# ALVI-Labs/frankenstein

Measured on AMD Instinct MI355X. Metric: neural frames/sec (train fwd+bwd+AdamW, whole job), higher is better.
Workload: dtype bf16; 1 GPU; brainformer-small (6L d=384 6x64 heads, N=6144 tokens) + 2-block perceiver, L1 head; fwd+bwd+clip+AdamW; per_gpu_batch=32, global_batch=32, frames_T=600, electrodes=256, parallelism=dp1, weights=random-init (seed 42)

## Files before the change

### frankenstein_amd/_lib.py

```python
from __future__ import annotations

import ctypes as C
from pathlib import Path

import os

LIB_PATH = Path(os.environ.get("FRANKEN_HIP_LIB") or Path(__file__).resolve().parent / "libfranken_hip.so")

FK_F32, FK_BF16 = 0, 1
MASK_NONE, MASK_CAUSAL, MASK_BLOCK_CAUSAL, MASK_PREFIX, MASK_KEYPAD, MASK_DENSE = 0, 1, 2, 3, 4, 5
NORM_LAYER, NORM_RMS = 0, 1
ATTN_Q_PRESCALED = 1

_p, _i64, _int, _f32, _f64, _sz, _u32 = C.c_void_p, C.c_int64, C.c_int, C.c_float, C.c_double, C.c_size_t, C.c_uint32

SIGNATURES = {
    "fk_version": (_int, []),
    "fk_last_error": (C.c_char_p, []),
    "fk_gemm_nt": (_int, [_p, _i64, _p, _i64, _p, _i64, _i64, _i64, _i64, _p, _p, _i64, _i64, _int, _int, _p]),
    "fk_gemm_nt_rope": (_int, [_p, _i64, _p, _i64, _p, _i64, _i64, _i64, _i64, _p, _p, _i64, _i64, _i64, _i64, _i64, _i64, _i64, _int, _p]),
    "fk_gemm_nt_swiglu": (_int, [_p, _i64, _p, _i64, _p, _i64, _p, _i64, _i64, _i64, _i64, _int, _p]),
    "fk_gemm_nt_dswiglu": (_int, [_p, _i64, _p, _i64, _p, _i64, _p, _i64, _i64, _i64, _i64, _int, _p]),
    "fk_mlp_bwd_fused": (_int, [_p, _i64, _p, _i64, _p, _i64, _p, _i64, _p, _i64, _p, _i64, _i64, _i64, _i64, _int, _p]),
    "fk_gemm_tn_workspace_bytes": (_sz, [_i64, _i64, _i64, _int]),
    "fk_gemm_tn": (_int, [_p, _i64, _p, _i64, _p, _i64, _i64, _i64, _i64, _int, _int, _p, _sz, _p]),
    "fk_colsum_workspace_bytes": (_sz, [_i64, _i64]),
    "fk_colsum": (_int, [_p, _i64, _p, _i64, _i64, _int, _int, _p, _sz, _p]),
    "fk_attn_fwd": (_int, [_p, _p, _p, _p, _p] + [_i64] * 13 + [_int, _i64, _i64, _i64, _p, _p, _f32, _int, _int, _p]),
    "fk_attn_bwd": (_int, [_p] * 10 + [_i64] * 13 + [_int, _i64, _i64, _i64, _p, _p, _f32, _p, _i64, _i64, _int, _int, _p]),
    "fk_attn_fwd_dropout": (_int, [_p, _p, _p, _p, _p] + [_i64] * 13 + [_int, _i64, _i64, _i64, _p, _p, _f32, _int, _f32, _p, _u32, _int, _p]),
    "fk_attn_bwd_dropout": (_int, [_p] * 10 + [_i64] * 13 + [_int, _i64, _i64, _i64, _p, _p, _f32, _p, _i64, _i64, _int, _f32, _p, _u32, _int, _p]),
    "fk_dropout": (_int, [_p, _p, _p, _i64, _f32, _p, _u32, _int, _p]),
    "fk_norm_fwd": (_int, [_p, _p, _p, _p, _p, _p, _i64, _i64, _f32, _int, _int, _p]),
    "fk_norm_bwd_workspace_bytes": (_sz, [_i64, _i64]),
    "fk_norm_bwd": (_int, [_p] * 9 + [_i64, _i64, _int, _int, _int, _p, _sz, _p]),
    "fk_rope": (_int, [_p, _i64, _i64, _i64, _i64, _i64, _p, _i64, _i64, _int, _int, _p]),
    "fk_patchify": (_int, [_p, _p, _i64, _i64, _i64, _i64, _i64, _int, _p]),
    "fk_swiglu_fwd": (_int, [_p, _p, _i64, _i64, _int, _p]),
    "fk_swiglu_bwd": (_int, [_p, _p, _p, _i64, _i64, _int, _p]),
    "fk_gelu_fwd": (_int, [_p, _p, _i64, _int, _p]),
    "fk_gelu_bwd": (_int, [_p, _p, _p, _i64, _int, _p]),
    "fk_cast_pack": (_int, [_p, _i64, _p, _i64, _i64, _i64, _int, _int, _p]),
    "fk_cast_pack_rows": (_int, [_p, _i64, _p, _i64, _i64, _i64, _int, _i64, _i64, _i64, _int, _p]),
    "fk_cast_pack_multi": (_int, [_p, _i64, _i64, _int, _p]),
    "fk_cast": (_int, [_p, _int, _p, _int, _i64, _p]),
# ... 68 lines not shown
```

### frankenstein_amd/csrc/mlp_fused.hip

```cpp
#include "fk_common.h"
#include <stdlib.h>

namespace {

#include "gemm_tile.h"

typedef __attribute__((address_space(3))) void lds_void_t;
typedef __attribute__((address_space(1))) const void glb_void_t;

struct MlpBwdArgs {
  const bf16_t* dy; const bf16_t* w2t; const bf16_t* h13; const bf16_t* w13t;
  bf16_t* dh13; bf16_t* dx;
  int64_t lddy, ldw2t, ldh, ldw13t, lddh, lddx;
  int M, H;
};

#ifndef MF_SPREAD
#define MF_SPREAD 1
#endif
#ifndef MF_SPREAD_ST
#define MF_SPREAD_ST 0
#endif
#ifndef MF_NT_DH13
#define MF_NT_DH13 1
// ... 449 lines not shown

  char* stg = smem + wave * 32 * MF_ROWP;
#pragma unroll
  for (int t = 0; t < MF_D / 32; ++t)
#pragma unroll
    for (int g = 0; g < 4; ++g) {
      bf16x4 v;
#pragma unroll
      for (int e = 0; e < 4; ++e) v[e] = (T)dx[t][4 * g + e];
      *reinterpret_cast<bf16x4*>(stg + li * MF_ROWP + (32 * t + 8 * g + 4 * lh) * 2) = v;
    }
  asm volatile("s_waitcnt lgkmcnt(0)" ::: "memory");
  if (lane < MF_D / 8) {
    for (int r = 0; r < 32; ++r) {
      const bf16x8 v = *reinterpret_cast<const bf16x8*>(stg + r * MF_ROWP + lane * 16);
      fk_st<true>(reinterpret_cast<bf16x8*>(p.dx + (int64_t)(m0w + r) * p.lddx + lane * 8), v);
    }
  }
  MF_ST(9)
  MF_ST_FLUSH
}


struct MlpUpArgs {
  const bf16_t* x; const bf16_t* w13; bf16_t* h13; bf16_t* g;
  int64_t ldx, ldw, ldh, ldg;
  int M, H;
};
constexpr int MU_NW = 8, MU_TOK = MU_NW * 32;
constexpr int MU_TILE = MF_KT * 32 * ROW_BYTES;
constexpr int MU_SLOT = 2 * MU_TILE;
constexpr int MU_HT = 32 * ROW_BYTES, MU_GT = 32 * 64;
constexpr int MU_LDS = 2 * MU_SLOT + MU_NW * (MU_HT + MU_GT);
static_assert(MU_LDS <= 160 * 1024, "LDS of a CU");
constexpr int MU_PIECES = MU_SLOT / 1024 / MU_NW;

__global__ __launch_bounds__(MU_NW * 64, 2) void mlp_up_fused_kernel(MlpUpArgs p) {
  extern __shared__ __attribute__((aligned(16))) char smem[];
  using T = bf16_t;
  const int tid = threadIdx.x, lane = tid & 63, li = lane & 31, lh = lane >> 5;
  const int wave = __builtin_amdgcn_readfirstlane(tid >> 6);
  const int m0w = blockIdx.x * MU_TOK + wave * 32;
  const int m = m0w + li, mc = m < p.M ? m : p.M - 1;
  const bool wave_full = m0w + 32 <= p.M;
  const int nchunks = p.H / 32, last = nchunks - 1;
  const int row8 = lane >> 3, ch = lane & 7;
  const unsigned lds0 = (unsigned)(uintptr_t)(lds_void_t*)smem;

  unsigned woff[MU_PIECES];
#pragma unroll
  for (int j = 0; j < MU_PIECES; ++j) {
    const int q = wave * MU_PIECES + j, tile = q / 24, s6 = (q % 24) >> 2, n = (q & 3) * 8 + row8;
    const int wrow = 8 * (n >> 2) + (n & 3) + 4 * tile;
    woff[j] = (unsigned)((wrow * (int)p.ldw + s6 * 64 + ((ch ^ ((n >> 1) & 7)) << 3)) * 2);
  }
  auto issue_w = [&](int c, int slot) __attribute__((always_inline)) {
    const void* gw = p.w13 + (int64_t)c * 64 * p.ldw;
    const unsigned d0 = __builtin_amdgcn_readfirstlane(lds0 + slot * MU_SLOT + wave * (MU_SLOT / MU_NW));
#pragma unroll
    for (int j = 0; j < MU_PIECES; ++j) mf_dma(gw, woff[j], d0 + j * 1024);
  };
  char* htile = smem + 2 * MU_SLOT + wave * (MU_HT + MU_GT);
  char* gtile = htile + MU_HT;
  T* hdst[4];
  T* gdst[2];
  bool hok[4], gok[2];
#pragma unroll
  for (int j = 0; j < 4; ++j) {
    const int mr = m0w + j * 8 + row8;
    hok[j] = mr < p.M;
    hdst[j] = p.h13 + (int64_t)(hok[j] ? mr : p.M - 1) * p.ldh + (ch << 3);
  }
#pragma unroll
  for (int j = 0; j < 2; ++j) {
    const int mr = m0w + j * 16 + (lane >> 2);
    gok[j] = mr < p.M;
    gdst[j] = p.g + (int64_t)(gok[j] ? mr : p.M - 1) * p.ldg + ((lane & 3) << 3);
  }

  issue_w(0, 0);
  Frag<T> xf[MF_D / 16];
  const T* xrow = p.x + (int64_t)mc * p.ldx + 8 * lh;
#pragma unroll
  for (int t = 0; t < MF_D / 16; ++t) frag_load_contig<T>(xf[t], xrow + 16 * t);
  asm volatile("s_waitcnt vmcnt(0)\n\ts_barrier" ::: "memory");

  bf16x8 rbh[4] = {}, rbg[2] = {};
  for (int c = 0; c < nchunks; ++c) {
    const char* t0 = smem + (c & 1) * MU_SLOT;
    const char* t1 = t0 + MU_TILE;
    if (c > 0) {
      if (wave_full) {
#pragma unroll
        for (int j = 0; j < 4; ++j) fk_st<true>(reinterpret_cast<bf16x8*>(hdst[j] + (c - 1) * 64), rbh[j]);
#pragma unroll
        for (int j = 0; j < 2; ++j) fk_st<true>(reinterpret_cast<bf16x8*>(gdst[j] + (c - 1) * 32), rbg[j]);
      } else {
#pragma unroll
        for (int j = 0; j < 4; ++j)
          if (hok[j]) fk_st<true>(reinterpret_cast<bf16x8*>(hdst[j] + (c - 1) * 64), rbh[j]);
#pragma unroll
        for (int j = 0; j < 2; ++j)
          if (gok[j]) fk_st<true>(reinterpret_cast<bf16x8*>(gdst[j] + (c - 1) * 32), rbg[j]);
      }
    }
    issue_w(c + 1 < nchunks ? c + 1 : last, (c + 1) & 1);
    f32x16 a1, a3;
#pragma unroll
// ... 43 lines not shown
    }
    asm volatile("s_waitcnt vmcnt(0)\n\ts_barrier" ::: "memory");
  }
  if (wave_full) {
#pragma unroll
    for (int j = 0; j < 4; ++j) fk_st<true>(reinterpret_cast<bf16x8*>(hdst[j] + last * 64), rbh[j]);
#pragma unroll
    for (int j = 0; j < 2; ++j) fk_st<true>(reinterpret_cast<bf16x8*>(gdst[j] + last * 32), rbg[j]);
  } else {
#pragma unroll
    for (int j = 0; j < 4; ++j)
      if (hok[j]) fk_st<true>(reinterpret_cast<bf16x8*>(hdst[j] + last * 64), rbh[j]);
#pragma unroll
    for (int j = 0; j < 2; ++j)
      if (gok[j]) fk_st<true>(reinterpret_cast<bf16x8*>(gdst[j] + last * 32), rbg[j]);
  }
}


struct QkvArgs {
  const bf16_t* x; const bf16_t* w; bf16_t* out; const float* table;
  int64_t ldx, ldw, ldo, table_bs, q_off;
  int M, N, T, pos_off, rot_chunks, q_chunks;
};
constexpr int QK_LDS = 2 * MU_SLOT + MU_NW * MU_HT;
static_assert(QK_LDS <= 160 * 1024, "LDS of a CU");

__global__ __launch_bounds__(MU_NW * 64, 2) void qkv_rope_fused_kernel(QkvArgs p) {
  extern __shared__ __attribute__((aligned(16))) char smem[];
  using T = bf16_t;
  const int tid = threadIdx.x, lane = tid & 63, li = lane & 31, lh = lane >> 5;
  const int wave = __builtin_amdgcn_readfirstlane(tid >> 6);
  const int m0w = blockIdx.x * MU_TOK + wave * 32;
  const int m = m0w + li, mc = m < p.M ? m : p.M - 1;
  const bool wave_full = m0w + 32 <= p.M;
  const int nchunks = p.N / 64, last = nchunks - 1;
  const int row8 = lane >> 3, ch = lane & 7;
  const unsigned lds0 = (unsigned)(uintptr_t)(lds_void_t*)smem;

  unsigned woff[MU_PIECES];
#pragma unroll
  for (int j = 0; j < MU_PIECES; ++j) {
    const int q = wave * MU_PIECES + j, tile = q / 24, s6 = (q % 24) >> 2, n = (q & 3) * 8 + row8;
    woff[j] = (unsigned)(((32 * tile + n) * (int)p.ldw + s6 * 64 + ((ch ^ ((n >> 1) & 7)) << 3)) * 2);
  }
  auto issue_w = [&](int c, int slot) __attribute__((always_inline)) {
    const void* gw = p.w + (int64_t)c * 64 * p.ldw;
    const unsigned d0 = __builtin_amdgcn_readfirstlane(lds0 + slot * MU_SLOT + wave * (MU_SLOT / MU_NW));
#pragma unroll
    for (int j = 0; j < MU_PIECES; ++j) mf_dma(gw, woff[j], d0 + j * 1024);
  };
  char* htile = smem + 2 * MU_SLOT + wave * MU_HT;
  T* odst[4];
  bool ook[4];
#pragma unroll
  for (int j = 0; j < 4; ++j) {
    const int mr = m0w + j * 8 + row8;
    ook[j] = mr < p.M;
    odst[j] = p.out + (int64_t)(ook[j] ? mr : p.M - 1) * p.ldo + (ch << 3);
  }
  const float* trow = p.table + (int64_t)(mc / p.T) * p.table_bs + (int64_t)(p.pos_off + mc % p.T) * 64 + 4 * lh;

  issue_w(0, 0);
  Frag<T> xf[MF_D / 16];
  const T* xrow = p.x + (int64_t)mc * p.ldx + 8 * lh;
#pragma unroll
  for (int t = 0; t < MF_D / 16; ++t) frag_load_contig<T>(xf[t], xrow + 16 * t);
  asm volatile("s_waitcnt vmcnt(0)\n\ts_barrier" ::: "memory");

  bf16x8 rb[4] = {};
  for (int c = 0; c < nchunks; ++c) {
    const char* t0 = smem + (c & 1) * MU_SLOT;
    const char* t1 = t0 + MU_TILE;
    if (c > 0) {
      if (wave_full) {
#pragma unroll
        for (int j = 0; j < 4; ++j) fk_st<true>(reinterpret_cast<bf16x8*>(odst[j] + (c - 1) * 64), rb[j]);
      } else {
#pragma unroll
        for (int j = 0; j < 4; ++j)
          if (ook[j]) fk_st<true>(reinterpret_cast<bf16x8*>(odst[j] + (c - 1) * 64), rb[j]);
      }
    }
    const bool rot = c < p.rot_chunks;
    f32x4 cs[8];
    if (rot) {
      const float* tq = trow + (c < p.q_chunks ? p.q_off : (int64_t)0);
      asm volatile("global_load_dwordx4 %0, %8, off\n\tglobal_load_dwordx4 %1, %8, off offset:32\n\t"
                   "global_load_dwordx4 %2, %8, off offset:64\n\tglobal_load_dwordx4 %3, %8, off offset:96\n\t"
                   "global_load_dwordx4 %4, %8, off offset:128\n\tglobal_load_dwordx4 %5, %8, off offset:160\n\t"
                   "global_load_dwordx4 %6, %8, off offset:192\n\tglobal_load_dwordx4 %7, %8, off offset:224"
// ... 44 lines not shown
#pragma unroll
    for (int j = 0; j < 4; ++j) rb[j] = *reinterpret_cast<const bf16x8*>(htile + nt_off(j * 8 + row8, ch));
    asm volatile("s_waitcnt vmcnt(0)\n\ts_barrier" ::: "memory");
  }
  if (wave_full) {
#pragma unroll
    for (int j = 0; j < 4; ++j) fk_st<true>(reinterpret_cast<bf16x8*>(odst[j] + last * 64), rb[j]);
  } else {
#pragma unroll
    for (int j = 0; j < 4; ++j)
      if (ook[j]) fk_st<true>(reinterpret_cast<bf16x8*>(odst[j] + last * 64), rb[j]);
  }
}

}

static bool mu_grid_fills(int64_t M) {
  const int64_t wg = fk_cdiv(M, MU_TOK), rounds = fk_cdiv(wg, 256);
  return wg * 10 >= rounds * 256 * 7;
}
bool fk_qkv_rope_fused_ok(int64_t M, int64_t N, int64_t K, int64_t lda, int64_t ldb, int64_t ldc, const void* bias, int64_t T, int64_t D, int64_t rot_cols,
                          int64_t q_cols, int dtype) {
  static const bool off = getenv("FK_QKV_FUSED") != nullptr && getenv("FK_QKV_FUSED")[0] == '0';
  return !off && dtype == FK_BF16 && K == MF_D && D == 64 && N % 64 == 0 && rot_cols % 64 == 0 && q_cols % 64 == 0 && rot_cols <= N && !bias && mu_grid_fills(M) &&
         M < (1LL << 31) && T > 0 && M % T == 0 && lda % 8 == 0 && ldb % 8 == 0 && ldc % 8 == 0 && 64 * ldb * 2 < (1LL << 32);
}
int fk_qkv_rope_fused_launch(const void* A, int64_t lda, const void* W, int64_t ldb, void* C, int64_t ldc, int64_t M, int64_t N, const float* table,
                             int64_t table_bs, int64_t T, int64_t pos_off, int64_t rot_cols, int64_t q_cols, int64_t q_off, void* stream) {
  QkvArgs a{(const bf16_t*)A, (const bf16_t*)W, (bf16_t*)C, table, lda, ldb, ldc, table_bs, q_off, (int)M, (int)N, (int)T, (int)pos_off,
            (int)(rot_cols / 64), (int)(q_cols / 64)};
  static bool once = (hipFuncSetAttribute(reinterpret_cast<const void*>(qkv_rope_fused_kernel), hipFuncAttributeMaxDynamicSharedMemorySize, QK_LDS) == hipSuccess);
  (void)once;
  hipLaunchKernelGGL(qkv_rope_fused_kernel, dim3((unsigned)fk_cdiv(M, MU_TOK)), dim3(MU_NW * 64), QK_LDS, (hipStream_t)stream, a);
  FK_CHECK_LAUNCH("fk_gemm_nt_rope (token-on-the-lane kernel)");
  return FK_OK;
}

bool fk_mlp_up_fused_ok(int64_t M, int64_t H, int64_t K, int64_t lda, int64_t ldb, int64_t ldh, int64_t ldg, int dtype) {
  static const bool off = getenv("FK_MLP_UP_FUSED") != nullptr && getenv("FK_MLP_UP_FUSED")[0] == '0';
  return !off && dtype == FK_BF16 && K == MF_D && H % 32 == 0 && mu_grid_fills(M) && M < (1LL << 31) && lda % 8 == 0 && ldb % 8 == 0 && ldh % 8 == 0 && ldg % 8 == 0 &&
         64 * ldb * 2 < (1LL << 32);
}
int fk_mlp_up_fused_launch(const void* A, int64_t lda, const void* W13, int64_t ldb, void* H13, int64_t ldh, void* G, int64_t ldg, int64_t M, int64_t H,
                           void* stream) {
  MlpUpArgs a{(const bf16_t*)A, (const bf16_t*)W13, (bf16_t*)H13, (bf16_t*)G, lda, ldb, ldh, ldg, (int)M, (int)H};
  static bool once = (hipFuncSetAttribute(reinterpret_cast<const void*>(mlp_up_fused_kernel), hipFuncAttributeMaxDynamicSharedMemorySize, MU_LDS) == hipSuccess);
  (void)once;
  hipLaunchKernelGGL(mlp_up_fused_kernel, dim3((unsigned)fk_cdiv(M, MU_TOK)), dim3(MU_NW * 64), MU_LDS, (hipStream_t)stream, a);
  FK_CHECK_LAUNCH("fk_gemm_nt_swiglu (token-on-the-lane kernel)");
  return FK_OK;
}

#ifdef MF_STAMP
extern "C" int fk_debug_mf_stamps(unsigned long long* out, int reset) {
  hipDeviceSynchronize();
  hipMemcpyFromSymbol(out, HIP_SYMBOL(mf_stamp_acc), sizeof(unsigned long long) * 16);
  if (reset) { unsigned long long z[16] = {0}; hipMemcpyToSymbol(HIP_SYMBOL(mf_stamp_acc), z, sizeof(z)); }
  return 0;
}
#endif

extern "C" int fk_mlp_bwd_fused(const void* dY, int64_t lddy, const void* W2T, int64_t ldw2t, const void* H13, int64_t ldh, const void* W13T,
                                int64_t ldw13t, void* dH13, int64_t lddh, void* dX, int64_t lddx, int64_t M, int64_t H, int64_t D, int dtype,
                                void* stream) {
  FK_CHECK_ARG(dtype == FK_BF16, "fk_mlp_bwd_fused: bf16 only (dtype %d)", dtype);
  FK_CHECK_ARG(D == MF_D, "fk_mlp_bwd_fused: model dimension %lld (built for %d)", (long long)D, MF_D);
  FK_CHECK_ARG(M > 0 && M < (1LL << 31) && H > 0 && H % 32 == 0 && H < (1 << 24), "fk_mlp_bwd_fused: bad shape M=%lld H=%lld", (long long)M, (long long)H);
  FK_CHECK_ARG(dY && W2T && H13 && W13T && dH13 && dX, "fk_mlp_bwd_fused: null pointer");
  FK_CHECK_ARG(lddy % 8 == 0 && ldw2t % 8 == 0 && ldh % 8 == 0 && ldw13t % 8 == 0 && lddh % 8 == 0 && lddx % 8 == 0 && lddy >= D && ldw2t >= D &&
                   ldh >= 2 * H && lddh >= 2 * H && ldw13t >= 2 * H && lddx >= D,
               "fk_mlp_bwd_fused: leading dimensions must be multiples of 8 elements and cover their rows");
  FK_CHECK_ARG(M * ldh * 2 < (1LL << 32) && (int64_t)D * ldw13t * 2 < (1LL << 32) && 32 * ldw2t * 2 < (1LL << 32),
               "fk_mlp_bwd_fused: the h13 block must be addressable with 32-bit byte offsets (M * ldh < 2^31 elements)");
// ... 16 lines not shown
```

### frankenstein_amd/engine.py

```python
from __future__ import annotations

from typing import List, Optional, Sequence, Tuple

import math
import os
import weakref

import torch

from . import kernels as K
from .kernels import Mask, NO_MASK

Tensor = torch.Tensor

_COMPUTE_DTYPE = torch.bfloat16
_EPOCH = 0


def set_compute_dtype(dtype) -> None:
    global _COMPUTE_DTYPE
    if isinstance(dtype, str):
        dtype = {"bf16": torch.bfloat16, "bfloat16": torch.bfloat16, "fp32": torch.float32, "float32": torch.float32}[dtype]
    assert dtype in (torch.bfloat16, torch.float32)
    _COMPUTE_DTYPE = dtype
# ... 319 lines not shown
class Dropout(torch.autograd.Function):

    @staticmethod
    def forward(ctx, x, drop):
        ctx.drop = drop
        return K.dropout(x.contiguous(), drop[0], drop[1], drop[2])

    @staticmethod
    def backward(ctx, dy):
        d = ctx.drop
        return K.dropout(dy.contiguous(), d[0], d[1], d[2]), None


class AttnBranch(torch.autograd.Function):

    @staticmethod
    def forward(ctx, x, ln_w, ln_b, pw, pb, qkv_b, spec, *qkv_w):
        H, D, mask, rope, residual, eps, nkind = spec[:7]
        drop = spec[7] if len(spec) > 7 else None
        B, N, d = x.shape
        M = B * N
        x2 = x.view(M, d)
        has_ln = ln_w is not None
        if has_ln:
            h, mean, rstd = K.norm_fwd(x2, ln_w.detach(), None if ln_b is None else ln_b.detach(), eps, nkind)
        else:
            h, mean, rstd = x2, None, None
        HD = H * D
        bq = None if qkv_b is None else shadow([qkv_b])
        prescale = False
        if rope is not None and D % 8 == 0 and (3 * HD) % 8 == 0:
            prescale = _attn_prescale(D) and mask.kind != K.MASK_DENSE and drop is None
            if prescale:
                tab, qtab = rope.pair((1.0 / math.sqrt(D)) * 1.4426950408889634)
                qkv = K.gemm_nt_rope(h, shadow(qkv_w), bq, tab, N, rope.pos_off(N), D, 2 * HD, q_cols=HD, q_table=qtab)
            else:
                qkv = K.gemm_nt_rope(h, shadow(qkv_w), bq, rope.table, N, rope.pos_off(N), D, 2 * HD)
            qkv3 = qkv.view(B, N, 3 * HD)
        elif (rope is None and N >= 64 and M % 8 == 0 and (3 * HD) % 8 == 0 and _attn_prescale(D) and mask.kind != K.MASK_DENSE and drop is None
              and os.environ.get("FK_ATTN_NO_IDENT_PRESCALE") is None):
            tab, qtab = identity_pair(D, (1.0 / math.sqrt(D)) * 1.4426950408889634, x.device)
            qkv = K.gemm_nt_rope(h, shadow(qkv_w), bq, tab, 8, 0, D, 2 * HD, q_cols=HD, q_table=qtab)
            qkv3 = qkv.view(B, N, 3 * HD)
            prescale = True
        else:
            qkv = K.gemm_nt(h, shadow(qkv_w), bias=bq)
            qkv3 = qkv.view(B, N, 3 * HD)
            if rope is not None:
                K.rope_(qkv3, 2 * H, D, rope.table, rope.pos_off(N))
        q, k, v = (qkv3[..., i * HD:(i + 1) * HD].unflatten(-1, (H, D)) for i in range(3))
        o, lse = K.attn_fwd(q, k, v, mask, q_prescaled=prescale, dropout=None if drop is None else drop[:3])
        if drop is None:
            y = K.gemm_nt(o.view(M, HD), shadow([pw]), bias=None if pb is None else shadow([pb]),
                          residual=x2 if residual else None)
        else:
            y = K.gemm_nt(o.view(M, HD), shadow([pw]), bias=None if pb is None else shadow([pb]))
            K.dropout(y, drop[0], drop[1], drop[3], residual=x2 if residual else None, out=y)
        ctx.spec, ctx.has_ln, ctx.nw, ctx.prescale = spec, has_ln, len(qkv_w), prescale
        ctx.flags = (ln_b is not None, pb is not None, qkv_b is not None)
        ctx.ln_b = ln_b
        ctx.save_for_backward(x, ln_w, pw, *qkv_w, h if has_ln else None, mean, rstd, qkv, o, lse)
        return y.view(B, N, -1)

    @staticmethod
    def backward(ctx, dy):
# ... 107 lines not shown
                       do.view(B, T, H, D), lse, dq.view(B, T, H, D), dkv3[..., :HD].unflatten(-1, (H, D)),
                       dkv3[..., HD:].unflatten(-1, (H, D)), mask)
        dh = K.gemm_nt(dq, shadow([qw], transpose=True))
        (dqw,) = wgrad(dq, h, [qw])
        dctx = K.gemm_nt(dkv, shadow([kw, vw], transpose=True))
        dkw, dvw = wgrad(dkv, c2, [kw, vw])
        dx, dg, db = norm_bwd(dh, x2, ln_w, ctx.ln_b, mean, rstd, dres=dy2)
        return dx.view(B, T, d), dctx.view(B, Nc, d), dg, db, dqw, dkw, dvw, dpw, None


_MLP_BWD_FUSED = os.environ.get("FK_MLP_BWD_FUSED", "1") != "0"


class MlpBranch(torch.autograd.Function):

    @staticmethod
    def forward(ctx, x, ln_w, ln_b, up_w, up_b, gate_w, down_w, down_b, spec):
        residual, eps, nkind = spec[:3]
        drop = spec[3] if len(spec) > 3 else None
        shp = x.shape
        d = shp[-1]
        x2 = x.reshape(-1, d)
        has_ln = ln_w is not None
        if has_ln:
            h, mean, rstd = K.norm_fwd(x2, ln_w.detach(), None if ln_b is None else ln_b.detach(), eps, nkind)
        else:
            h, mean, rstd = x2, None, None
        fused = gate_w is not None and up_b is None and up_w.shape[0] % 8 == 0
        if fused:
            a, g = K.gemm_nt_swiglu(h, shadow_swiglu(up_w, gate_w))
        else:
            ups = [up_w] if gate_w is None else [up_w, gate_w]
            a = K.gemm_nt(h, shadow(ups), bias=None if up_b is None else shadow([up_b]))
            g = K.gelu_fwd(a) if gate_w is None else K.swiglu_fwd(a)
        if drop is None:
            y = K.gemm_nt(g, shadow([down_w]), bias=None if down_b is None else shadow([down_b]),
                          residual=x2 if residual else None)
        else:
            y = K.gemm_nt(g, shadow([down_w]), bias=None if down_b is None else shadow([down_b]))
            K.dropout(y, drop[0], drop[1], drop[2], residual=x2 if residual else None, out=y)
        ctx.spec, ctx.has_ln, ctx.fused = spec, has_ln, fused
        ctx.flags = (ln_b is not None, up_b is not None, gate_w is not None, down_b is not None)
        ctx.ln_b = ln_b
        ctx.save_for_backward(x, ln_w, up_w, gate_w, down_w, h if has_ln else None, mean, rstd, a, g)
        return y.view(*shp[:-1], y.shape[-1])

    @staticmethod
    def backward(ctx, dy):
        residual, eps, nkind = ctx.spec[:3]
        drop = ctx.spec[3] if len(ctx.spec) > 3 else None
        x, ln_w, up_w, gate_w, down_w, h, mean, rstd, a, g = ctx.saved_tensors
        has_lnb, has_ub, gated, has_db = ctx.flags
        shp = x.shape
        d = shp[-1]
        x2 = x.reshape(-1, d)
        if h is None:
            h = x2
# ... 408 lines not shown
```

### frankenstein_amd/kernels.py

```python
from __future__ import annotations

import math
from typing import Optional, Tuple

import torch

from . import _lib
from ._lib import FK_BF16, FK_F32, MASK_BLOCK_CAUSAL, MASK_CAUSAL, MASK_DENSE, MASK_KEYPAD, MASK_NONE, MASK_PREFIX, NORM_LAYER, NORM_RMS, ATTN_Q_PRESCALED, call, lib

Tensor = torch.Tensor


TIMERS = None
TIMER_PREFIX = None


class _timed:
    __slots__ = ("name", "ev")

    def __init__(self, name):
        self.name = name

    def __enter__(self):
        self.ev = None
# ... 72 lines not shown
    q_off = 0
    if q_table is not None and q_cols:
        assert q_table.shape == table.shape and q_table.dtype == torch.float32 and q_table.is_contiguous() and q_table.stride() == table.stride()
        q_off = (q_table.data_ptr() - table.data_ptr()) // 4
    else:
        q_cols = 0
    with _timed(f"gemm_nt_rope:{M}x{N}x{Kd}"):
        call("fk_gemm_nt_rope", a.data_ptr(), a.stride(0), w.data_ptr(), w.stride(0), out.data_ptr(), N, M, N, Kd, _ptr(bias),
             table.data_ptr(), tbs, T, pos_off, D, rot_cols, q_cols, q_off, fk_dtype(a), _stream())
    return out


def gemm_nt_swiglu(a: Tensor, w13: Tensor) -> Tuple[Tensor, Tensor]:
    assert a.dim() == 2 and w13.dim() == 2 and a.shape[1] == w13.shape[1] and a.dtype == w13.dtype
    assert a.stride(1) == 1 and w13.is_contiguous()
    M, Kd = a.shape
    H = w13.shape[0] // 2
    h13 = torch.empty((M, 2 * H), dtype=a.dtype, device=a.device)
    g = torch.empty((M, H), dtype=a.dtype, device=a.device)
    with _timed(f"gemm_nt_swiglu:{M}x{2 * H}x{Kd}"):
        call("fk_gemm_nt_swiglu", a.data_ptr(), a.stride(0), w13.data_ptr(), w13.stride(0), h13.data_ptr(), 2 * H,
             g.data_ptr(), H, M, H, Kd, fk_dtype(a), _stream())
    return h13, g


def gemm_nt_dswiglu(dy: Tensor, w2t: Tensor, h13: Tensor) -> Tensor:
    assert dy.dim() == 2 and w2t.dim() == 2 and dy.shape[1] == w2t.shape[1] and dy.dtype == w2t.dtype == h13.dtype
    assert dy.stride(1) == 1 and w2t.is_contiguous() and h13.is_contiguous()
    M, Kd = dy.shape
    H = w2t.shape[0]
    assert h13.shape == (M, 2 * H)
    dh13 = torch.empty_like(h13)
    with _timed(f"gemm_nt_dswiglu:{M}x{H}x{Kd}"):
        call("fk_gemm_nt_dswiglu", dy.data_ptr(), dy.stride(0), w2t.data_ptr(), w2t.stride(0), h13.data_ptr(), 2 * H,
             dh13.data_ptr(), 2 * H, M, H, Kd, fk_dtype(dy), _stream())
    return dh13


def mlp_bwd_fused(dy: Tensor, w2t: Tensor, h13: Tensor, w13t: Tensor) -> Tuple[Tensor, Tensor]:
    M, d = dy.shape
    H = w2t.shape[0]
    assert dy.dtype == torch.bfloat16 == w2t.dtype == h13.dtype == w13t.dtype and dy.stride(1) == 1
    assert w2t.shape == (H, d) and w2t.is_contiguous() and h13.shape == (M, 2 * H) and h13.is_contiguous() and w13t.shape == (d, 2 * H) and w13t.is_contiguous()
    dh13 = torch.empty_like(h13)
    dx = torch.empty((M, d), dtype=dy.dtype, device=dy.device)
    with _timed(f"mlp_bwd_fused:{M}x{H}x{d}"):
# ... 567 lines not shown
```

### include/franken_hip.h

```cpp
#ifndef FRANKEN_HIP_H
#define FRANKEN_HIP_H

#include <stddef.h>
#include <stdint.h>

#ifdef __cplusplus
extern "C" {
#endif

#define FK_VERSION 302

#define FK_OK 0
#define FK_EINVAL (-1)
#define FK_ELAUNCH (-2)
#define FK_EUNSUPPORTED (-3)

enum { FK_F32 = 0, FK_BF16 = 1 };
enum { FK_MASK_NONE = 0, FK_MASK_CAUSAL = 1, FK_MASK_BLOCK_CAUSAL = 2, FK_MASK_PREFIX = 3, FK_MASK_KEYPAD = 4, FK_MASK_DENSE = 5 };
enum { FK_ATTN_Q_PRESCALED = 1 };
enum { FK_NORM_LAYER = 0, FK_NORM_RMS = 1 };
enum { FK_ACT_SWIGLU = 0, FK_ACT_GELU = 1 };

int fk_version(void);
const char* fk_last_error(void);

int fk_gemm_nt(const void* A, int64_t lda, const void* B, int64_t ldb, void* C, int64_t ldc, int64_t M, int64_t N,
               int64_t K, const void* bias, const void* residual, int64_t ldr, int64_t res_rows, int dtype,
               int out_dtype, void* stream);
int fk_gemm_nt_rope(const void* A, int64_t lda, const void* B, int64_t ldb, void* C, int64_t ldc, int64_t M, int64_t N,
                    int64_t K, const void* bias, const float* table, int64_t table_bs, int64_t T, int64_t pos_off, int64_t D,
                    int64_t rot_cols, int64_t q_cols, int64_t q_table_off, int dtype, void* stream);
int fk_gemm_nt_swiglu(const void* A, int64_t lda, const void* W13, int64_t ldb, void* H13, int64_t ldh, void* G,
                      int64_t ldg, int64_t M, int64_t H, int64_t K, int dtype, void* stream);
int fk_gemm_nt_dswiglu(const void* dY, int64_t lda, const void* W2T, int64_t ldb, const void* H13, int64_t ldh, void* dH13,
                       int64_t lddh, int64_t M, int64_t H, int64_t K, int dtype, void* stream);
int fk_mlp_bwd_fused(const void* dY, int64_t lddy, const void* W2T, int64_t ldw2t, const void* H13, int64_t ldh, const void* W13T,
                     int64_t ldw13t, void* dH13, int64_t lddh, void* dX, int64_t lddx, int64_t M, int64_t H, int64_t D, int dtype,
                     void* stream);
size_t fk_gemm_tn_workspace_bytes(int64_t M, int64_t N1, int64_t N2, int dtype);
int fk_gemm_tn(const void* A, int64_t lda, const void* B, int64_t ldb, float* C, int64_t ldc, int64_t M, int64_t N1,
               int64_t N2, int accumulate, int dtype, void* workspace, size_t workspace_bytes, void* stream);
size_t fk_colsum_workspace_bytes(int64_t rows, int64_t cols);
int fk_colsum(const void* X, int64_t ld, float* out, int64_t rows, int64_t cols, int accumulate, int dtype,
              void* workspace, size_t workspace_bytes, void* stream);

int fk_attn_fwd(const void* Q, const void* K, const void* V, void* O, float* LSE, int64_t B, int64_t H, int64_t Nq,
                int64_t Nk, int64_t D, int64_t q_bs, int64_t q_rs, int64_t k_bs, int64_t k_rs, int64_t v_bs,
                int64_t v_rs, int64_t o_bs, int64_t o_rs, int mask_kind, int64_t mask_c, int64_t q_off, int64_t k_off,
                const int32_t* limits, const int32_t* qfirst, float scale, int flags, int dtype, void* stream);
int fk_attn_bwd(const void* Q, const void* K, const void* V, const void* O, const void* dO, const float* LSE,
                void* dQ, void* dK, void* dV, float* delta_ws, int64_t B, int64_t H, int64_t Nq, int64_t Nk, int64_t D,
                int64_t q_bs, int64_t q_rs, int64_t k_bs, int64_t k_rs, int64_t v_bs, int64_t v_rs, int64_t o_bs,
                int64_t o_rs, int mask_kind, int64_t mask_c, int64_t q_off, int64_t k_off, const int32_t* limits,
                const int32_t* qfirst, float scale, const float* rope_table, int64_t rope_bs, int64_t rope_off, int flags,
                int dtype, void* stream);

int fk_attn_fwd_dropout(const void* Q, const void* K, const void* V, void* O, float* LSE, int64_t B, int64_t H, int64_t Nq,
                        int64_t Nk, int64_t D, int64_t q_bs, int64_t q_rs, int64_t k_bs, int64_t k_rs, int64_t v_bs,
// ... 118 lines not shown
```

Baseline: 393,400 frames/s.

## Fuse pre-norm LayerNorm/RMSNorm into QKV-rope and SwiGLU up-projection kernels

Adds templated LN variants of the token-on-the-lane QKV+rope and MLP up-projection kernels. Each one computes mean/rstd and the normalized activations in registers as a prologue, writes h/mean/rstd for backward, and feeds the normalized fragments straight into the GEMM. The engine routes pre-norm attention and SwiGLU MLP through these entry points when the input is contiguous. This removes a separate norm kernel launch and the re-read of h by the GEMM, at the cost of extra register and LDS pressure in the GEMM prologue.

```diff
diff --git a/frankenstein_amd/_lib.py b/frankenstein_amd/_lib.py
--- a/frankenstein_amd/_lib.py
+++ b/frankenstein_amd/_lib.py
@@ -21,6 +21,8 @@
     "fk_gemm_nt_rope": (_int, [_p, _i64, _p, _i64, _p, _i64, _i64, _i64, _i64, _p, _p, _i64, _i64, _i64, _i64, _i64, _i64, _i64, _int, _p]),
     "fk_gemm_nt_swiglu": (_int, [_p, _i64, _p, _i64, _p, _i64, _p, _i64, _i64, _i64, _i64, _int, _p]),
     "fk_gemm_nt_dswiglu": (_int, [_p, _i64, _p, _i64, _p, _i64, _p, _i64, _i64, _i64, _i64, _int, _p]),
+    "fk_norm_gemm_nt_rope": (_int, [_p, _p, _p, _f32, _int, _p, _p, _p, _p, _i64, _p, _i64, _i64, _i64, _i64, _p, _p, _i64, _i64, _i64, _i64, _i64, _i64, _i64, _int, _p]),
+    "fk_norm_gemm_nt_swiglu": (_int, [_p, _p, _p, _f32, _int, _p, _p, _p, _p, _i64, _p, _i64, _p, _i64, _i64, _i64, _i64, _int, _p]),
     "fk_mlp_bwd_fused": (_int, [_p, _i64, _p, _i64, _p, _i64, _p, _i64, _p, _i64, _p, _i64, _i64, _i64, _i64, _int, _p]),
     "fk_gemm_tn_workspace_bytes": (_sz, [_i64, _i64, _i64, _int]),
     "fk_gemm_tn": (_int, [_p, _i64, _p, _i64, _p, _i64, _i64, _i64, _i64, _int, _int, _p, _sz, _p]),
diff --git a/frankenstein_amd/csrc/mlp_fused.hip b/frankenstein_amd/csrc/mlp_fused.hip
--- a/frankenstein_amd/csrc/mlp_fused.hip
+++ b/frankenstein_amd/csrc/mlp_fused.hip
@@ -495,10 +495,101 @@
 }
 
 
+struct NormIn {
+  const float* gamma; const float* beta; bf16_t* h; float* mean; float* rstd;
+  float eps; int kind;
+};
+
+FK_DEV void mu_norm_params(const NormIn& n, int lane, f32x4 (&gb)[3]) {
+#pragma unroll
+  for (int r = 0; r < 3; ++r) {
+    const int q = lane + 64 * r;
+    gb[r] = f32x4{0.0f, 0.0f, 0.0f, 0.0f};
+    if (q < MF_D / 4) gb[r] = *reinterpret_cast<const f32x4*>(n.gamma + 4 * q);
+    else if (n.beta) gb[r] = *reinterpret_cast<const f32x4*>(n.beta + 4 * (q - MF_D / 4));
+  }
+}
+
+FK_DEV void mu_norm_prologue(Frag<bf16_t> (&xf)[MF_D / 16], const NormIn& n, const f32x4 (&gb)[3], char* tile, int lane, int m0w, int M) {
+  using T = bf16_t;
+  const int li = lane & 31, lh = lane >> 5, row8 = lane >> 3, ch = lane & 7;
+#pragma unroll
+  for (int r = 0; r < 3; ++r) *reinterpret_cast<f32x4*>(tile + 16 * (lane + 64 * r)) = gb[r];
+  const float inv = 1.0f / MF_D;
+  float s[8];
+#pragma unroll
+  for (int j = 0; j < 8; ++j) {
+    float a = 0.0f;
+#pragma unroll
+    for (int k = 0; k < 3; ++k)
+#pragma unroll
+      for (int i = 0; i < 8; ++i) a += (float)xf[j + 8 * k].v[i];
+    s[j] = a;
+  }
+#pragma unroll
+  for (int t = 0; t < MF_D / 16; ++t) asm volatile("" : "+v"(xf[t].v));
+  float c = ((s[0] + s[4]) + (s[2] + s[6])) + ((s[1] + s[5]) + (s[3] + s[7]));
+  const float mu = n.kind == FK_NORM_LAYER ? (c + __shfl_xor(c, 32, 64)) * inv : 0.0f;
+#pragma unroll
+  for (int j = 0; j < 8; ++j) {
+    float a = 0.0f;
+#pragma unroll
+    for (int k = 0; k < 3; ++k)
+#pragma unroll
+      for (int i = 0; i < 8; ++i) {
+        const float d = (float)xf[j + 8 * k].v[i] - mu;
+        a += d * d;
+      }
+    s[j] = a;
+  }
+#pragma unroll
+  for (int t = 0; t < MF_D / 16; ++t) asm volatile("" : "+v"(xf[t].v));
+  c = ((s[0] + s[4]) + (s[2] + s[6])) + ((s[1] + s[5]) + (s[3] + s[7]));
+  const float rs = rsqrtf((c + __shfl_xor(c, 32, 64)) * inv + n.eps);
+  const int m = m0w + li;
+  if (lh == 0 && m < M) {
+    if (n.mean) n.mean[m] = mu;
+    n.rstd[m] = rs;
+  }
+#pragma unroll
+  for (int t = 0; t < MF_D / 16; ++t) {
+    const char* gp = tile + (16 * t + 8 * lh) * 4;
+    const f32x4 g0 = *reinterpret_cast<const f32x4*>(gp), g1 = *reinterpret_cast<const f32x4*>(gp + 16);
+    const f32x4 b0 = *reinterpret_cast<const f32x4*>(gp + 4 * MF_D), b1 = *reinterpret_cast<const f32x4*>(gp + 4 * MF_D + 16);
+#pragma unroll
+    for (int i = 0; i < 8; ++i) {
+      float tt = ((float)xf[t].v[i] - mu) * rs;
+      if (n.kind == FK_NORM_RMS) tt = (float)(bf16_t)tt;
+      xf[t].v[i] = (T)(tt * (i < 4 ? g0[i] : g1[i - 4]) + (i < 4 ? b0[i] : b1[i - 4]));
+    }
+    if ((t & 3) == 3)
+      asm volatile("" : "+v"(xf[t - 3].v), "+v"(xf[t - 2].v), "+v"(xf[t - 1].v), "+v"(xf[t].v)::"memory");
+  }
+  T* hd[4];
+  bool hok[4];
+#pragma unroll
+  for (int j = 0; j < 4; ++j) {
+    const int mr = m0w + j * 8 + row8;
+    hok[j] = mr < M;
+    hd[j] = n.h + (int64_t)(hok[j] ? mr : M - 1) * MF_D + (ch << 3);
+  }
+#pragma unroll
+  for (int k = 0; k < MF_D / 64; ++k) {
+#pragma unroll
+    for (int tt = 0; tt < 4; ++tt) *reinterpret_cast<bf16x8*>(tile + nt_off(li, 2 * tt + lh)) = xf[4 * k + tt].v;
+#pragma unroll
+    for (int j = 0; j < 4; ++j) {
+      const bf16x8 v = *reinterpret_cast<const bf16x8*>(tile + nt_off(j * 8 + row8, ch));
+      if (hok[j]) fk_st<true>(reinterpret_cast<bf16x8*>(hd[j] + 64 * k), v);
+    }
+  }
+}
+
 struct MlpUpArgs {
   const bf16_t* x; const bf16_t* w13; bf16_t* h13; bf16_t* g;
   int64_t ldx, ldw, ldh, ldg;
   int M, H;
+  NormIn ln;
 };
 constexpr int MU_NW = 8, MU_TOK = MU_NW * 32;
 constexpr int MU_TILE = MF_KT * 32 * ROW_BYTES;
@@ -508,6 +599,7 @@
 static_assert(MU_LDS <= 160 * 1024, "LDS of a CU");
 constexpr int MU_PIECES = MU_SLOT / 1024 / MU_NW;
 
+template <bool LN>
 __global__ __launch_bounds__(MU_NW * 64, 2) void mlp_up_fused_kernel(MlpUpArgs p) {
   extern __shared__ __attribute__((aligned(16))) char smem[];
   using T = bf16_t;
@@ -552,11 +644,14 @@
   }
 
   issue_w(0, 0);
+  f32x4 gb[3];
+  if constexpr (LN) mu_norm_params(p.ln, lane, gb);
   Frag<T> xf[MF_D / 16];
   const T* xrow = p.x + (int64_t)mc * p.ldx + 8 * lh;
 #pragma unroll
   for (int t = 0; t < MF_D / 16; ++t) frag_load_contig<T>(xf[t], xrow + 16 * t);
   asm volatile("s_waitcnt vmcnt(0)\n\ts_barrier" ::: "memory");
+  if constexpr (LN) mu_norm_prologue(xf, p.ln, gb, htile, lane, m0w, p.M);
 
   bf16x8 rbh[4] = {}, rbg[2] = {};
   for (int c = 0; c < nchunks; ++c) {
@@ -646,10 +741,12 @@
   const bf16_t* x; const bf16_t* w; bf16_t* out; const float* table;
   int64_t ldx, ldw, ldo, table_bs, q_off;
   int M, N, T, pos_off, rot_chunks, q_chunks;
+  NormIn ln;
 };
 constexpr int QK_LDS = 2 * MU_SLOT + MU_NW * MU_HT;
 static_assert(QK_LDS <= 160 * 1024, "LDS of a CU");
 
+template <bool LN>
 __global__ __launch_bounds__(MU_NW * 64, 2) void qkv_rope_fused_kernel(QkvArgs p) {
   extern __shared__ __attribute__((aligned(16))) char smem[];
   using T = bf16_t;
@@ -686,11 +783,14 @@
   const float* trow = p.table + (int64_t)(mc / p.T) * p.table_bs + (int64_t)(p.pos_off + mc % p.T) * 64 + 4 * lh;
 
   issue_w(0, 0);
+  f32x4 gb[3];
+  if constexpr (LN) mu_norm_params(p.ln, lane, gb);
   Frag<T> xf[MF_D / 16];
   const T* xrow = p.x + (int64_t)mc * p.ldx + 8 * lh;
 #pragma unroll
   for (int t = 0; t < MF_D / 16; ++t) frag_load_contig<T>(xf[t], xrow + 16 * t);
   asm volatile("s_waitcnt vmcnt(0)\n\ts_barrier" ::: "memory");
+  if constexpr (LN) mu_norm_prologue(xf, p.ln, gb, htile, lane, m0w, p.M);
 
   bf16x8 rb[4] = {};
   for (int c = 0; c < nchunks; ++c) {
@@ -781,33 +881,84 @@
 bool fk_qkv_rope_fused_ok(int64_t M, int64_t N, int64_t K, int64_t lda, int64_t ldb, int64_t ldc, const void* bias, int64_t T, int64_t D, int64_t rot_cols,
                           int64_t q_cols, int dtype) {
   static const bool off = getenv("FK_QKV_FUSED") != nullptr && getenv("FK_QKV_FUSED")[0] == '0';
-  return !off && dtype == FK_BF16 && K == MF_D && D == 64 && N % 64 == 0 && rot_cols % 64 == 0 && q_cols % 64 == 0 && rot_cols <= N && !bias && mu_grid_fills(M) &&
-         M < (1LL << 31) && T > 0 && M % T == 0 && lda % 8 == 0 && ldb % 8 == 0 && ldc % 8 == 0 && 64 * ldb * 2 < (1LL << 32);
+  return !off && dtype == FK_BF16 && K == MF_D && D == 64 && N > 0 && N < (1LL << 31) && N % 64 == 0 && rot_cols % 64 == 0 && q_cols % 64 == 0 &&
+         rot_cols <= N && !bias && M > 0 && mu_grid_fills(M) && M < (1LL << 31) && T > 0 && M % T == 0 && lda % 8 == 0 && ldb % 8 == 0 && ldc % 8 == 0 &&
+         lda >= K && ldb >= K && ldc >= N && 64 * ldb * 2 < (1LL << 32);
+}
+template <bool LN> static int qkv_launch(const QkvArgs& a, void* stream) {
+  static bool once = (hipFuncSetAttribute(reinterpret_cast<const void*>(qkv_rope_fused_kernel<LN>), hipFuncAttributeMaxDynamicSharedMemorySize, QK_LDS) == hipSuccess);
+  (void)once;
+  hipLaunchKernelGGL(qkv_rope_fused_kernel<LN>, dim3((unsigned)fk_cdiv(a.M, MU_TOK)), dim3(MU_NW * 64), QK_LDS, (hipStream_t)stream, a);
+  FK_CHECK_LAUNCH("fk_gemm_nt_rope (token-on-the-lane kernel)");
+  return FK_OK;
 }
 int fk_qkv_rope_fused_launch(const void* A, int64_t lda, const void* W, int64_t ldb, void* C, int64_t ldc, int64_t M, int64_t N, const float* table,
                              int64_t table_bs, int64_t T, int64_t pos_off, int64_t rot_cols, int64_t q_cols, int64_t q_off, void* stream) {
   QkvArgs a{(const bf16_t*)A, (const bf16_t*)W, (bf16_t*)C, table, lda, ldb, ldc, table_bs, q_off, (int)M, (int)N, (int)T, (int)pos_off,
-            (int)(rot_cols / 64), (int)(q_cols / 64)};
-  static bool once = (hipFuncSetAttribute(reinterpret_cast<const void*>(qkv_rope_fused_kernel), hipFuncAttributeMaxDynamicSharedMemorySize, QK_LDS) == hipSuccess);
-  (void)once;
-  hipLaunchKernelGGL(qkv_rope_fused_kernel, dim3((unsigned)fk_cdiv(M, MU_TOK)), dim3(MU_NW * 64), QK_LDS, (hipStream_t)stream, a);
-  FK_CHECK_LAUNCH("fk_gemm_nt_rope (token-on-the-lane kernel)");
-  return FK_OK;
+            (int)(rot_cols / 64), (int)(q_cols / 64), NormIn{}};
+  return qkv_launch<false>(a, stream);
 }
 
 bool fk_mlp_up_fused_ok(int64_t M, int64_t H, int64_t K, int64_t lda, int64_t ldb, int64_t ldh, int64_t ldg, int dtype) {
   static const bool off = getenv("FK_MLP_UP_FUSED") != nullptr && getenv("FK_MLP_UP_FUSED")[0] == '0';
-  return !off && dtype == FK_BF16 && K == MF_D && H % 32 == 0 && mu_grid_fills(M) && M < (1LL << 31) && lda % 8 == 0 && ldb % 8 == 0 && ldh % 8 == 0 && ldg % 8 == 0 &&
-         64 * ldb * 2 < (1LL << 32);
+  return !off && dtype == FK_BF16 && K == MF_D && H > 0 && H < (1LL << 30) && H % 32 == 0 && M > 0 && mu_grid_fills(M) && M < (1LL << 31) &&
+         lda % 8 == 0 && ldb % 8 == 0 && ldh % 8 == 0 && ldg % 8 == 0 && lda >= K && ldb >= K && ldh >= 2 * H && ldg >= H && 64 * ldb * 2 < (1LL << 32);
+}
+template <bool LN> static int mlp_up_launch(const MlpUpArgs& a, void* stream) {
+  static bool once = (hipFuncSetAttribute(reinterpret_cast<const void*>(mlp_up_fused_kernel<LN>), hipFuncAttributeMaxDynamicSharedMemorySize, MU_LDS) == hipSuccess);
+  (void)once;
+  hipLaunchKernelGGL(mlp_up_fused_kernel<LN>, dim3((unsigned)fk_cdiv(a.M, MU_TOK)), dim3(MU_NW * 64), MU_LDS, (hipStream_t)stream, a);
+  FK_CHECK_LAUNCH("fk_gemm_nt_swiglu (token-on-the-lane kernel)");
+  return FK_OK;
 }
 int fk_mlp_up_fused_launch(const void* A, int64_t lda, const void* W13, int64_t ldb, void* H13, int64_t ldh, void* G, int64_t ldg, int64_t M, int64_t H,
                            void* stream) {
-  MlpUpArgs a{(const bf16_t*)A, (const bf16_t*)W13, (bf16_t*)H13, (bf16_t*)G, lda, ldb, ldh, ldg, (int)M, (int)H};
-  static bool once = (hipFuncSetAttribute(reinterpret_cast<const void*>(mlp_up_fused_kernel), hipFuncAttributeMaxDynamicSharedMemorySize, MU_LDS) == hipSuccess);
-  (void)once;
-  hipLaunchKernelGGL(mlp_up_fused_kernel, dim3((unsigned)fk_cdiv(M, MU_TOK)), dim3(MU_NW * 64), MU_LDS, (hipStream_t)stream, a);
-  FK_CHECK_LAUNCH("fk_gemm_nt_swiglu (token-on-the-lane kernel)");
-  return FK_OK;
+  MlpUpArgs a{(const bf16_t*)A, (const bf16_t*)W13, (bf16_t*)H13, (bf16_t*)G, lda, ldb, ldh, ldg, (int)M, (int)H, NormIn{}};
+  return mlp_up_launch<false>(a, stream);
+}
+
+static bool ln_env_off(const char* name) {
+  const char* all = getenv("FK_LN_FUSED");
+  const char* one = getenv(name);
+  return (all != nullptr && all[0] == '0') || (one != nullptr && one[0] == '0');
+}
+static bool ln_fused_ok(bool off, const void* X, const float* gamma, const float* beta, const void* Hn, const float* mean, const float* rstd, int64_t K,
+                        float eps, int kind, int dtype) {
+  return !off && dtype == FK_BF16 && K == MF_D && (kind == FK_NORM_LAYER || kind == FK_NORM_RMS) && X && gamma && Hn && rstd &&
+         (kind == FK_NORM_RMS || mean) && (((uintptr_t)X | (uintptr_t)gamma | (uintptr_t)beta | (uintptr_t)Hn) & 15) == 0;
+}
+
+extern "C" int fk_norm_gemm_nt_rope(const void* X, const float* gamma, const float* beta, float eps, int kind, void* Hn, float* mean, float* rstd,
+                                    const void* B, int64_t ldb, void* C, int64_t ldc, int64_t M, int64_t N, int64_t K, const void* bias,
+                                    const float* table, int64_t table_bs, int64_t T, int64_t pos_off, int64_t D, int64_t rot_cols, int64_t q_cols,
+                                    int64_t q_table_off, int dtype, void* stream) {
+  static const bool off = ln_env_off("FK_LN_QKV_FUSED");
+  FK_CHECK_ARG(table && T > 0 && D > 0 && rot_cols >= 0, "fk_norm_gemm_nt_rope: bad rope arguments");
+  FK_CHECK_ARG(q_cols >= 0 && q_cols <= rot_cols && q_cols % 8 == 0 && q_table_off % 4 == 0, "fk_norm_gemm_nt_rope: bad pre-scaled query table");
+  if (ln_fused_ok(off, X, gamma, beta, Hn, mean, rstd, K, eps, kind, dtype) && B && C && (((uintptr_t)B | (uintptr_t)C | (uintptr_t)table) & 15) == 0 &&
+      pos_off >= 0 && fk_qkv_rope_fused_ok(M, N, K, K, ldb, ldc, bias, T, D, rot_cols, q_cols, dtype)) {
+    QkvArgs a{(const bf16_t*)X, (const bf16_t*)B, (bf16_t*)C, table, K, ldb, ldc, table_bs, q_table_off, (int)M, (int)N, (int)T, (int)pos_off,
+              (int)(rot_cols / 64), (int)(q_cols / 64), NormIn{gamma, beta, (bf16_t*)Hn, mean, rstd, eps, kind}};
+    return qkv_launch<true>(a, stream);
+  }
+  const int r = fk_norm_fwd(X, gamma, beta, Hn, mean, rstd, M, K, eps, kind, dtype, stream);
+  if (r != FK_OK) return r;
+  return fk_gemm_nt_rope(Hn, K, B, ldb, C, ldc, M, N, K, bias, table, table_bs, T, pos_off, D, rot_cols, q_cols, q_table_off, dtype, stream);
+}
+
+extern "C" int fk_norm_gemm_nt_swiglu(const void* X, const float* gamma, const float* beta, float eps, int kind, void* Hn, float* mean, float* rstd,
+                                      const void* W13, int64_t ldb, void* H13, int64_t ldh, void* G, int64_t ldg, int64_t M, int64_t H, int64_t K,
+                                      int dtype, void* stream) {
+  static const bool off = ln_env_off("FK_LN_UP_FUSED");
+  if (ln_fused_ok(off, X, gamma, beta, Hn, mean, rstd, K, eps, kind, dtype) && W13 && H13 && G &&
+      (((uintptr_t)W13 | (uintptr_t)H13 | (uintptr_t)G) & 15) == 0 && fk_mlp_up_fused_ok(M, H, K, K, ldb, ldh, ldg, dtype)) {
+    MlpUpArgs a{(const bf16_t*)X, (const bf16_t*)W13, (bf16_t*)H13, (bf16_t*)G, K, ldb, ldh, ldg, (int)M, (int)H,
+                NormIn{gamma, beta, (bf16_t*)Hn, mean, rstd, eps, kind}};
+    return mlp_up_launch<true>(a, stream);
+  }
+  const int r = fk_norm_fwd(X, gamma, beta, Hn, mean, rstd, M, K, eps, kind, dtype, stream);
+  if (r != FK_OK) return r;
+  return fk_gemm_nt_swiglu(Hn, K, W13, ldb, H13, ldh, G, ldg, M, H, K, dtype, stream);
 }
 
 #ifdef MF_STAMP
diff --git a/frankenstein_amd/engine.py b/frankenstein_amd/engine.py
--- a/frankenstein_amd/engine.py
+++ b/frankenstein_amd/engine.py
@@ -365,25 +365,34 @@
         M = B * N
         x2 = x.view(M, d)
         has_ln = ln_w is not None
-        if has_ln:
-            h, mean, rstd = K.norm_fwd(x2, ln_w.detach(), None if ln_b is None else ln_b.detach(), eps, nkind)
-        else:
-            h, mean, rstd = x2, None, None
         HD = H * D
         bq = None if qkv_b is None else shadow([qkv_b])
+        rope_path = rope is not None and D % 8 == 0 and (3 * HD) % 8 == 0
+        ident_path = (not rope_path and rope is None and N >= 64 and M % 8 == 0 and (3 * HD) % 8 == 0 and _attn_prescale(D)
+                      and mask.kind != K.MASK_DENSE and drop is None and os.environ.get("FK_ATTN_NO_IDENT_PRESCALE") is None)
+        if has_ln and (rope_path or ident_path) and x2.is_contiguous():
+            def rope_proj(*a, **kw):
+                return K.norm_gemm_nt_rope(x2, ln_w.detach(), None if ln_b is None else ln_b.detach(), eps, nkind, shadow(qkv_w), bq, *a, **kw)
+        else:
+            if has_ln:
+                h, mean, rstd = K.norm_fwd(x2, ln_w.detach(), None if ln_b is None else ln_b.detach(), eps, nkind)
+            else:
+                h, mean, rstd = x2, None, None
+
+            def rope_proj(*a, **kw):
+                return h, mean, rstd, K.gemm_nt_rope(h, shadow(qkv_w), bq, *a, **kw)
         prescale = False
-        if rope is not None and D % 8 == 0 and (3 * HD) % 8 == 0:
+        if rope_path:
             prescale = _attn_prescale(D) and mask.kind != K.MASK_DENSE and drop is None
             if prescale:
                 tab, qtab = rope.pair((1.0 / math.sqrt(D)) * 1.4426950408889634)
-                qkv = K.gemm_nt_rope(h, shadow(qkv_w), bq, tab, N, rope.pos_off(N), D, 2 * HD, q_cols=HD, q_table=qtab)
+                h, mean, rstd, qkv = rope_proj(tab, N, rope.pos_off(N), D, 2 * HD, q_cols=HD, q_table=qtab)
             else:
-                qkv = K.gemm_nt_rope(h, shadow(qkv_w), bq, rope.table, N, rope.pos_off(N), D, 2 * HD)
+                h, mean, rstd, qkv = rope_proj(rope.table, N, rope.pos_off(N), D, 2 * HD)
             qkv3 = qkv.view(B, N, 3 * HD)
-        elif (rope is None and N >= 64 and M % 8 == 0 and (3 * HD) % 8 == 0 and _attn_prescale(D) and mask.kind != K.MASK_DENSE and drop is None
-              and os.environ.get("FK_ATTN_NO_IDENT_PRESCALE") is None):
+        elif ident_path:
             tab, qtab = identity_pair(D, (1.0 / math.sqrt(D)) * 1.4426950408889634, x.device)
-            qkv = K.gemm_nt_rope(h, shadow(qkv_w), bq, tab, 8, 0, D, 2 * HD, q_cols=HD, q_table=qtab)
+            h, mean, rstd, qkv = rope_proj(tab, 8, 0, D, 2 * HD, q_cols=HD, q_table=qtab)
             qkv3 = qkv.view(B, N, 3 * HD)
             prescale = True
         else:
@@ -537,17 +546,21 @@
         d = shp[-1]
         x2 = x.reshape(-1, d)
         has_ln = ln_w is not None
-        if has_ln:
-            h, mean, rstd = K.norm_fwd(x2, ln_w.detach(), None if ln_b is None else ln_b.detach(), eps, nkind)
-        else:
-            h, mean, rstd = x2, None, None
         fused = gate_w is not None and up_b is None and up_w.shape[0] % 8 == 0
-        if fused:
-            a, g = K.gemm_nt_swiglu(h, shadow_swiglu(up_w, gate_w))
-        else:
-            ups = [up_w] if gate_w is None else [up_w, gate_w]
-            a = K.gemm_nt(h, shadow(ups), bias=None if up_b is None else shadow([up_b]))
-            g = K.gelu_fwd(a) if gate_w is None else K.swiglu_fwd(a)
+        if has_ln and fused and x2.is_contiguous():
+            h, mean, rstd, a, g = K.norm_gemm_nt_swiglu(x2, ln_w.detach(), None if ln_b is None else ln_b.detach(), eps, nkind,
+                                                        shadow_swiglu(up_w, gate_w))
+        else:
+            if has_ln:
+                h, mean, rstd = K.norm_fwd(x2, ln_w.detach(), None if ln_b is None else ln_b.detach(), eps, nkind)
+            else:
+                h, mean, rstd = x2, None, None
+            if fused:
+                a, g = K.gemm_nt_swiglu(h, shadow_swiglu(up_w, gate_w))
+            else:
+                ups = [up_w] if gate_w is None else [up_w, gate_w]
+                a = K.gemm_nt(h, shadow(ups), bias=None if up_b is None else shadow([up_b]))
+                g = K.gelu_fwd(a) if gate_w is None else K.swiglu_fwd(a)
         if drop is None:
             y = K.gemm_nt(g, shadow([down_w]), bias=None if down_b is None else shadow([down_b]),
                           residual=x2 if residual else None)
diff --git a/frankenstein_amd/kernels.py b/frankenstein_amd/kernels.py
--- a/frankenstein_amd/kernels.py
+++ b/frankenstein_amd/kernels.py
@@ -118,6 +118,50 @@
         call("fk_gemm_nt_swiglu", a.data_ptr(), a.stride(0), w13.data_ptr(), w13.stride(0), h13.data_ptr(), 2 * H,
              g.data_ptr(), H, M, H, Kd, fk_dtype(a), _stream())
     return h13, g
+
+
+def _norm_out(x2: Tensor, gamma: Tensor, beta: Optional[Tensor]):
+    assert x2.dim() == 2 and x2.is_contiguous() and gamma.dtype == torch.float32 and gamma.is_contiguous()
+    assert beta is None or (beta.dtype == torch.float32 and beta.is_contiguous())
+    rows = x2.shape[0]
+    h = torch.empty_like(x2)
+    return h, torch.empty(rows, dtype=torch.float32, device=x2.device), torch.empty(rows, dtype=torch.float32, device=x2.device)
+
+
+def norm_gemm_nt_rope(x: Tensor, gamma: Tensor, beta: Optional[Tensor], eps: float, kind: int, w: Tensor, bias: Optional[Tensor],
+                      table: Tensor, T: int, pos_off: int, D: int, rot_cols: int, q_cols: int = 0, q_table: Optional[Tensor] = None):
+    assert x.dim() == 2 and w.dim() == 2 and x.shape[1] == w.shape[1] and x.dtype == w.dtype and w.stride(1) == 1
+    assert table.dtype == torch.float32 and table.is_contiguous() and table.shape[-1] == 2 and table.shape[-2] == D // 2
+    M, Kd = x.shape
+    N = w.shape[0]
+    tbs = table.stride(0) if table.dim() == 4 else 0
+    assert pos_off >= 0 and pos_off + T <= table.shape[-3] and M % T == 0
+    h, mean, rstd = _norm_out(x, gamma, beta)
+    out = torch.empty((M, N), dtype=x.dtype, device=x.device)
+    q_off = 0
+    if q_table is not None and q_cols:
+        assert q_table.shape == table.shape and q_table.dtype == torch.float32 and q_table.is_contiguous() and q_table.stride() == table.stride()
+        q_off = (q_table.data_ptr() - table.data_ptr()) // 4
+    else:
+        q_cols = 0
+    with _timed(f"norm_gemm_nt_rope:{M}x{N}x{Kd}"):
+        call("fk_norm_gemm_nt_rope", x.data_ptr(), gamma.data_ptr(), _ptr(beta), eps, kind, h.data_ptr(), mean.data_ptr(), rstd.data_ptr(),
+             w.data_ptr(), w.stride(0), out.data_ptr(), N, M, N, Kd, _ptr(bias), table.data_ptr(), tbs, T, pos_off, D, rot_cols, q_cols, q_off,
+             fk_dtype(x), _stream())
+    return h, mean, rstd, out
+
+
+def norm_gemm_nt_swiglu(x: Tensor, gamma: Tensor, beta: Optional[Tensor], eps: float, kind: int, w13: Tensor):
+    assert x.dim() == 2 and w13.dim() == 2 and x.shape[1] == w13.shape[1] and x.dtype == w13.dtype and w13.is_contiguous()
+    M, Kd = x.shape
+    H = w13.shape[0] // 2
+    h, mean, rstd = _norm_out(x, gamma, beta)
+    h13 = torch.empty((M, 2 * H), dtype=x.dtype, device=x.device)
+    g = torch.empty((M, H), dtype=x.dtype, device=x.device)
+    with _timed(f"norm_gemm_nt_swiglu:{M}x{2 * H}x{Kd}"):
+        call("fk_norm_gemm_nt_swiglu", x.data_ptr(), gamma.data_ptr(), _ptr(beta), eps, kind, h.data_ptr(), mean.data_ptr(), rstd.data_ptr(),
+             w13.data_ptr(), w13.stride(0), h13.data_ptr(), 2 * H, g.data_ptr(), H, M, H, Kd, fk_dtype(x), _stream())
+    return h, mean, rstd, h13, g
 
 
 def gemm_nt_dswiglu(dy: Tensor, w2t: Tensor, h13: Tensor) -> Tensor:
diff --git a/include/franken_hip.h b/include/franken_hip.h
--- a/include/franken_hip.h
+++ b/include/franken_hip.h
@@ -34,6 +34,13 @@
                       int64_t ldg, int64_t M, int64_t H, int64_t K, int dtype, void* stream);
 int fk_gemm_nt_dswiglu(const void* dY, int64_t lda, const void* W2T, int64_t ldb, const void* H13, int64_t ldh, void* dH13,
                        int64_t lddh, int64_t M, int64_t H, int64_t K, int dtype, void* stream);
+int fk_norm_gemm_nt_rope(const void* X, const float* gamma, const float* beta, float eps, int kind, void* Hn, float* mean, float* rstd,
+                         const void* B, int64_t ldb, void* C, int64_t ldc, int64_t M, int64_t N, int64_t K, const void* bias,
+                         const float* table, int64_t table_bs, int64_t T, int64_t pos_off, int64_t D, int64_t rot_cols, int64_t q_cols,
+                         int64_t q_table_off, int dtype, void* stream);
+int fk_norm_gemm_nt_swiglu(const void* X, const float* gamma, const float* beta, float eps, int kind, void* Hn, float* mean, float* rstd,
+                           const void* W13, int64_t ldb, void* H13, int64_t ldh, void* G, int64_t ldg, int64_t M, int64_t H, int64_t K,
+                           int dtype, void* stream);
 int fk_mlp_bwd_fused(const void* dY, int64_t lddy, const void* W2T, int64_t ldw2t, const void* H13, int64_t ldh, const void* W13T,
                      int64_t ldw13t, void* dH13, int64_t lddh, void* dX, int64_t lddx, int64_t M, int64_t H, int64_t D, int dtype,
                      void* stream);
```

Result: no change. 394,100 frames/s, median of 6 (+0.2%).
